# emiliofidalgo/liodom

Hardware: AMD Instinct MI355X
Metric: scans/sec (64×1800 cloud, prev_frames=20) at 1 GPU; pose RMSE vs CPU ref (higher is better)
Workload: dtype f64

## Files before the change

### liodom_amd/csrc/kernels_knn.h

```cpp
constexpr float kCellInv = 1.0f;
constexpr double kCellSize = 1.0;

struct Top5 {
  unsigned long long k0, k1, k2, k3, k4;
  int p0, p1, p2, p3, p4;
};
constexpr unsigned long long kTop5Empty = (0x7f800000ull << 32) | 0x7fffffffull;
__device__ __forceinline__ float top5_dist(unsigned long long k) { return __int_as_float((int)(k >> 32)); }
__device__ __forceinline__ int top5_index(unsigned long long k) { return (int)(unsigned int)(k & 0xFFFFFFFFull); }
#define TOP5_STAGE(K, P)                                          \
  {                                                               \
    const bool lt = ck < (K);                                     \
    const unsigned long long nk = lt ? ck : (K);                  \
    const int np = lt ? cp : (P);                                 \
    ck = lt ? (K) : ck;                                           \
    cp = lt ? (P) : cp;                                           \
    (K) = nk; (P) = np;                                           \
  }
__device__ __forceinline__ void top5_insert(Top5& t, float d, int wi, int pos) {
  unsigned long long ck = ((unsigned long long)(unsigned int)__float_as_int(d) << 32) | (unsigned int)wi;
  int cp = pos;
  if (ck < t.k4) {
    TOP5_STAGE(t.k0, t.p0)
    TOP5_STAGE(t.k1, t.p1)
// ... 125 lines not shown
      }
    }
    int adj[U];
#pragma unroll
    for (int u = 0; u < U; u++) adj[u] = s_adj[c[u]];
#pragma unroll
    for (int u = 0; u < U; u++) a[u] += adj[u];
    float4 m[U];
#pragma unroll
    for (int u = 0; u < U; u++) m[u] = sp[a[u]];
#pragma unroll
    for (int u = 0; u < U; u++)
      t.consider(i + u * kKnnGroup < T, sqdist_cand(qx, qy, qz, m[u]), __float_as_int(m[u].w), a[u]);
  }
  __builtin_amdgcn_wave_barrier();
  if (dbg && hl == 0) {
    dbg[0] = (unsigned int)(dbg_t1 - dbg_t0);
    dbg[1] = (unsigned int)(wall_clock64() - dbg_t1);
    dbg[2] = ((unsigned int)((T + U * kKnnGroup - 1) / (U * kKnnGroup)) << 16) | ((unsigned int)T << 20);
    dbg[3] = dbg_nseg;
  }
}

__device__ __forceinline__ bool best2_select(const Best2Acc& t, int hl, int half_shift, float& d5, int (&pos)[5]) {
  unsigned int v = (unsigned int)__float_as_int(t.m1), w = (unsigned int)__float_as_int(t.m2);
  int ph = t.p1, pn = t.p2;
  unsigned int g[6];
#pragma unroll
  for (int r = 0; r < 5; r++) {
    g[r] = half_min_u32(v);
    const unsigned int win = (unsigned int)((__ballot(v == g[r]) >> half_shift) & 0xFFFFFFFFull);
    const int l = __ffs(win) - 1;
    pos[r] = __shfl(ph, l, kKnnGroup);
    const bool mine = hl == l;
    v = mine ? w : v;
    w = mine ? 0x7f800000u : w;
    ph = mine ? pn : ph;
  }
  g[5] = half_min_u32(v);
  const unsigned int s3 = half_min_u32((unsigned int)__float_as_int(t.m3));
  const unsigned int one = 0x3f800000u;
  d5 = __int_as_float((int)g[4]);
  if (g[4] < one) return g[0] < g[1] && g[1] < g[2] && g[2] < g[3] && g[3] < g[4] && g[4] < g[5] && g[4] < s3;
  return s3 >= one;
}


__device__ __forceinline__ void knn_merge(Top5& t, Top5& g, int hl, int half_shift) {
  unsigned long long gk[5]; int gp[5];
#pragma unroll
  for (int r = 0; r < 5; r++) {
    const unsigned long long key = t.k0;
    const unsigned int dmin = half_min_u32((unsigned int)(key >> 32));
    unsigned int win = (unsigned int)((__ballot((unsigned int)(key >> 32) == dmin) >> half_shift) & 0xFFFFFFFFull);
    unsigned long long mk;
    if (__popc(win) == 1) {
      mk = ((unsigned long long)dmin << 32) | (unsigned int)__shfl((int)(unsigned int)(key & 0xFFFFFFFFull), __ffs(win) - 1, kKnnGroup);
    } else {
      mk = half_min_u64(key);
      win = (unsigned int)((__ballot(key == mk) >> half_shift) & 0xFFFFFFFFull);
    }
    const int wl = __ffs(win) - 1;
    gp[r] = __shfl(t.p0, wl, kKnnGroup);
    gk[r] = mk;
    if (hl == wl) {
      t.k0 = t.k1; t.k1 = t.k2; t.k2 = t.k3; t.k3 = t.k4; t.k4 = kTop5Empty;
      t.p0 = t.p1; t.p1 = t.p2; t.p2 = t.p3; t.p3 = t.p4; t.p4 = -1;
    }
  }
  g.k0 = gk[0]; g.k1 = gk[1]; g.k2 = gk[2]; g.k3 = gk[3]; g.k4 = gk[4];
  g.p0 = gp[0]; g.p1 = gp[1]; g.p2 = gp[2]; g.p3 = gp[3]; g.p4 = gp[4];
}

__device__ void rebuild_alloc(const DevView& v, int s, StreamState& st, int block, int nblocks);
__device__ void rebuild_count_and_pad(const DevView& v, int s, StreamState& st, int eb, int block, int* sbase, int* sslot, bool keep);

template <int kQ>
struct KnnShared {
  int incl[kQ][kKnnGroup];
  int adj[kQ][kKnnGroup];
  float nn[kQ][16];
  int res[kQ][4];
  double part[kQ][32];
  double blk[kQ][24];
};

__device__ __forceinline__ float best2_bound(const Best2Acc& t, int half_shift) {
  float B = 1.0f;
  const float thr[4] = {0.36f, 0.09f, 0.0225f, 0.0036f};
#pragma unroll
  for (int k = 0; k < 4; k++) {
    const int c = __popc((unsigned int)(__ballot(t.m1 <= thr[k]) >> half_shift)) + __popc((unsigned int)(__ballot(t.m2 <= thr[k]) >> half_shift));
    B = c >= 5 ? thr[k] : B;
  }
  return B;
}

template <class Tune>
__device__ __forceinline__ void knn_probe_cells(const DevView& v, const StreamState& st, int fc, int hl, int cx, int cy, int cz, float qx, float qy, float qz,
                                                const CellSlot* cells, const unsigned int* bits, unsigned int tmask,
                                                unsigned int& start, unsigned int& cnt, float& lb) {
  if (hl < 27) {
    const int dx = hl % 3 - 1, dy = (hl / 3) % 3 - 1, dz = hl / 9 - 1;
    const unsigned long long key = pack_cell(cx + dx, cy + dy, cz + dz);
    unsigned int h = hash_cell(key, tmask);
    if (Tune::kProbeBoth) {
      const unsigned int word = bits[h >> 5];
      const uint4 raw = *reinterpret_cast<const uint4*>(cells + h);
// ... 68 lines not shown
  const float r = fminf(sqrtf(pre.sq.w), 1.0f) + margin;
  const float B = r * r * (1.0f + 1e-5f);
  Top5Acc ta;
  {
    const unsigned long long sentinel = ((unsigned long long)(unsigned int)__float_as_int(B) << 32) | 0x7fffffffull;
    ta.t.k0 = ta.t.k1 = ta.t.k2 = ta.t.k3 = ta.t.k4 = sentinel;
    ta.t.p0 = ta.t.p1 = ta.t.p2 = ta.t.p3 = ta.t.p4 = -1;
  }
  const bool all = cnt > 0 && !(lb > B);
  knn_stream_cells<Top5Acc, 2, 2, 64>(ta, sp, sh.incl[grp], sh.adj[grp], start, all ? cnt : 0u, hl, qx, qy, qz);
  float gl = B;
  if (ta.t.p4 >= 0) gl = fminf(gl, top5_dist(ta.t.k4));
  pre.gsq = __int_as_float((int)half_min_u32((unsigned int)__float_as_int(gl)));
  pre.p[0] = ta.t.p0; pre.p[1] = ta.t.p1; pre.p[2] = ta.t.p2; pre.p[3] = ta.t.p3; pre.p[4] = ta.t.p4;
#pragma unroll
  for (int k = 0; k < 5; k++) pre.c[k] = sp[pre.p[k] >= 0 ? pre.p[k] : 0];
}

template <int kKnnThreads, bool kPre = false, bool kTail = true, bool kWt = kPre>
__device__ __forceinline__ void knn_block(const DevView& v, int s, StreamState& st, int fc, int outer_it, int eb, int bv, int E,
                                          KnnShared<kKnnThreads / kKnnGroup>& sh, const float4& p_in, const double (&T_in)[12],
                                          const KnnPre& pre, const double* qt) {
  constexpr int kKnnQueries = kKnnThreads / kKnnGroup;
  typedef KnnTune<(kKnnThreads >= 256)> Tune;
  const int grp = threadIdx.x / kKnnGroup;
  const int e = bv * kKnnQueries + grp;
  const int hl = threadIdx.x & (kKnnGroup - 1);
  const int half_shift = (threadIdx.x & 32);
  const bool dbgb = (bv == 5) && (s == 0) && (threadIdx.x == 0) && (outer_it == 0);
  const unsigned long long t_blk = (kInstrument && (v.debug & 32)) ? wall_clock64() : 0ull;
  DBG_STAMP(v, dbgb, 1, 0);
  bool active = e < E;
  float qx = 0.f, qy = 0.f, qz = 0.f;
  if (active) {
    float4 p = p_in;
    double T[12];
#pragma unroll
    for (int i = 0; i < 12; i++) T[i] = T_in[i];
    if (!Tune::kHoistLoads) {
      p = v.edges[((size_t)eb * v.n_streams + s) * v.edge_cap + e];
#pragma unroll
      for (int i = 0; i < 12; i++) T[i] = st.odom[i];
    }
    transform_point(T, p.x, p.y, p.z, &qx, &qy, &qz);
    if (v.knn_q && hl == 0) v.knn_q[((size_t)s * 2 + outer_it) * v.edge_cap + e] = make_float4(qx, qy, qz, 0.f);
    active = ld_isfinite((double)qx) && ld_isfinite((double)qy) && ld_isfinite((double)qz) &&
             fabsf(qx) < 1.0e9f && fabsf(qy) < 1.0e9f && fabsf(qz) < 1.0e9f;
  }
  DBG_STAMP(v, dbgb, 1, 1); DBG_QSTAMP(1);
  if (hl == 0) { sh.res[grp][0] = 0; sh.res[grp][1] = -1; sh.res[grp][2] = -1; }
  float d5 = __int_as_float(0x7f800000);
  if (active) {
    const int cx = (int)floorf(qx * kCellInv), cy = (int)floorf(qy * kCellInv), cz = (int)floorf(qz * kCellInv);
    const unsigned int tmask = st.table_mask;
    const int stab = s + LD_TAB_PARITY(v, fc) * v.n_streams;
    const CellSlot* cells = v.cells + (size_t)stab * v.table_size;
    const unsigned int* bits = v.cell_bits + (size_t)stab * (v.table_size >> 5);
    const float4* sp = v.sorted_pts + (size_t)stab * v.sorted_cap;
    float d5_r = __int_as_float(0x7f800000);
    int pos5[5] = {-1, -1, -1, -1, -1};
    bool reranked = false;
    if (kPre) {
      if ((kInstrument && (v.debug & 64)) && hl == 0 && !(pre.gsq > 0.f)) atomicAdd(&v.dbg_clk[262], 1ull);
      if (pre.gsq > 0.f) {
        Top5 t, g;
        top5_clear(t);
#pragma unroll
        for (int k = 0; k < 5; k++) {
          if (pre.p[k] >= 0) top5_insert(t, sqdist_f(qx, qy, qz, pre.c[k].x, pre.c[k].y, pre.c[k].z), __float_as_int(pre.c[k].w), pre.p[k]);
        }
        knn_merge(t, g, hl, half_shift);
        const float d5n = g.p4 >= 0 ? top5_dist(g.k4) : __int_as_float(0x7f800000);
        const double ddx = (double)qx - (double)pre.sq.x, ddy = (double)qy - (double)pre.sq.y, ddz = (double)qz - (double)pre.sq.z;
        const double delta = sqrt(ddx * ddx + ddy * ddy + ddz * ddz) * (1.0 + 1e-12);
        const double r = sqrt((double)pre.gsq) * (1.0 - 2e-7) - delta;
        double limit = r > 0.0 ? r * r * (1.0 - 1e-6) : 0.0;
        {
          const double cs = kCellSize;
          const double fx = (double)qx - (double)(int)floorf(pre.sq.x * kCellInv) * cs, fy = (double)qy - (double)(int)floorf(pre.sq.y * kCellInv) * cs,
                       fz = (double)qz - (double)(int)floorf(pre.sq.z * kCellInv) * cs;
          const double edge = fmin(fmin(fmin(fx, cs - fx), fmin(fy, cs - fy)), fmin(fz, cs - fz));
          const double ro = (cs + edge) * (1.0 - 2e-7);
          const double lo = ro > 0.0 ? ro * ro * (1.0 - 1e-6) : 0.0;
// ... 77 lines not shown
    Best2Acc b2;
    b2.clear();
    int dbg_n = 0;
    bool dbg_two_phase = false;
    {
      const bool now = pend && (have_b ? !(lb > B) : (hl == 13 || hl == 27 || lb <= Tune::kNearSq));
      if (kInstrument && (v.debug & 32)) dbg_n = __shfl(half_incl_scan_i32(now ? (int)cnt : 0), kKnnGroup - 1, kKnnGroup);
      knn_stream_cells<Best2Acc, Tune::kLoadsBig, Tune::kLoadsFlat, Tune::kBigCell, Tune::kCursor>(b2, sp, sh.incl[grp], sh.adj[grp], start, now ? cnt : 0u, hl, qx, qy, qz,
                                                                                     ((kInstrument && (v.debug & 32)) && s == 0 && e < E) ? v.dbg_q + ((size_t)outer_it * v.edge_cap + e) * 12 + 8 : nullptr);
      pend = pend && !now;
    }
    DBG_STAMP(v, dbgb, 1, 3); DBG_QSTAMP(3);
    if (!have_b && ((__ballot(pend) >> half_shift) & 0xFFFFFFFFull)) {
      B = best2_bound(b2, half_shift);
      pend = pend && !(lb > B);
      if ((__ballot(pend) >> half_shift) & 0xFFFFFFFFull) {
        if (kInstrument && (v.debug & 32)) { dbg_n += __shfl(half_incl_scan_i32(pend ? (int)cnt : 0), kKnnGroup - 1, kKnnGroup); dbg_two_phase = true; }
        knn_stream_cells<Best2Acc, Tune::kLoadsBig, Tune::kLoadsFlat, Tune::kBigCell, Tune::kCursor>(b2, sp, sh.incl[grp], sh.adj[grp], start, pend ? cnt : 0u, hl, qx, qy, qz);
      }
    } else {
      pend = false;
    }
    DBG_STAMP(v, dbgb, 1, 4); DBG_QSTAMP(4);
    const bool certain = best2_select(b2, hl, half_shift, d5, pos5) && !v.knn_exact_only;
    if ((kInstrument && (v.debug & 32)) && s == 0 && e < E && hl == 0) v.dbg_q[((size_t)outer_it * v.edge_cap + e) * 12] = (unsigned int)dbg_n | (dbg_two_phase ? 0x40000000u : 0u) | (certain ? 0u : 0x80000000u);
    if ((kInstrument && (v.debug & 64)) && hl == 0) {
      atomicAdd(&v.dbg_clk[256 + (certain ? 0 : 1)], 1ull);
      if (dbg_two_phase) atomicAdd(&v.dbg_clk[258], 1ull);
      atomicAdd(&v.dbg_clk[384 + (dbg_n / 64 < 63 ? dbg_n / 64 : 63)], 1ull);
    }
    if (!certain) {
      const bool all = cnt > 0 && (!(lb > B) || (!have_b && (hl == 13 || hl == 27 || lb <= Tune::kNearSq)));
      Top5Acc ta;
      Top5 g;
      {
        const float bnd = d5 < 1.0f ? d5 : 1.0f;
        const unsigned long long sentinel = ((unsigned long long)(unsigned int)__float_as_int(bnd) << 32) | 0x7fffffffull;
        ta.t.k0 = ta.t.k1 = ta.t.k2 = ta.t.k3 = ta.t.k4 = sentinel;
        ta.t.p0 = ta.t.p1 = ta.t.p2 = ta.t.p3 = ta.t.p4 = -1;
      }
      knn_stream_cells<Top5Acc, 2, 2, 64>(ta, sp, sh.incl[grp], sh.adj[grp], start, all ? cnt : 0u, hl, qx, qy, qz);
      knn_merge(ta.t, g, hl, half_shift);
      d5 = g.p4 >= 0 ? top5_dist(g.k4) : __int_as_float(0x7f800000);
      pos5[0] = g.p0; pos5[1] = g.p1; pos5[2] = g.p2; pos5[3] = g.p3; pos5[4] = g.p4;
    }
    if (outer_it == 0 && v.knn_save_pos && !(kWt && !kPre)) {
      const float sk = (cnt > 0 && !(!(lb > B) || (!have_b && (hl == 13 || hl == 27 || lb <= Tune::kNearSq)))) ? lb : __int_as_float(0x7f800000);
// ... 3 lines not shown
      float guard = __int_as_float((int)gd);
      {
        const float cs = (float)kCellSize;
        const float fx = qx - (float)cx * cs, fy = qy - (float)cy * cs, fz = qz - (float)cz * cs;
        float edge = fminf(fminf(fminf(fx, cs - fx), fminf(fy, cs - fy)), fminf(fz, cs - fz));
        edge = edge > 0.f ? edge : 0.f;
        const float outer = (cs + edge) * (cs + edge) * (1.0f - 1e-6f);
        guard = guard < outer ? guard : outer;
      }
      v.knn_save_pos[((size_t)s * v.edge_cap + e) * kKnnGroup + hl] = make_int2(b2.p1, b2.p2);
      if (hl == 0) v.knn_save_g[(size_t)s * v.edge_cap + e] = guard < 3.0e38f ? guard : 3.0e38f;
    }
    if ((kInstrument && (v.debug & 64)) && s == 0 && hl == 0) {
      const int bin = (int)((wall_clock64() - t_blk) / 100ull);
      atomicAdd(&v.dbg_clk[320 + (bin < 63 ? bin : 63)], 1ull);
      const int nb = dbg_n < 64 ? 0 : dbg_n < 128 ? 1 : dbg_n < 256 ? 2 : dbg_n < 512 ? 3 : dbg_n < 1024 ? 4 : 5;
      atomicAdd(&v.dbg_clk[448 + (bin / 4 < 7 ? bin / 4 : 7) * 8 + nb + (dbg_two_phase ? 0 : 0)], 1ull);
      if (!certain) atomicAdd(&v.dbg_clk[448 + (bin / 4 < 7 ? bin / 4 : 7) * 8 + 7], 1ull);
      if (dbg_two_phase) atomicAdd(&v.dbg_clk[448 + (bin / 4 < 7 ? bin / 4 : 7) * 8 + 6], 1ull);
    }
    }
    else d5 = d5_r;
    DBG_STAMP(v, dbgb, 1, 5); DBG_QSTAMP(5);
    if (d5 < 1.0f && !(kPre && reranked)) {
      const int mypos = hl == 0 ? pos5[0] : hl == 1 ? pos5[1] : hl == 2 ? pos5[2] : hl == 3 ? pos5[3] : pos5[4];
      if (hl < 5) {
        const float4 m = sp[mypos];
        sh.nn[grp][hl * 3 + 0] = m.x; sh.nn[grp][hl * 3 + 1] = m.y; sh.nn[grp][hl * 3 + 2] = m.z;
        if (hl < 2) sh.res[grp][1 + hl] = __float_as_int(m.w);
      }
      if (hl == 0) sh.res[grp][0] = 1;
    }
  }
  if (outer_it == 0 && v.knn_save_q && e < E && hl == 0) {
    v.knn_save_q[(size_t)s * v.edge_cap + e] = make_float4(qx, qy, qz, d5);
    if (!active && v.knn_save_g) v.knn_save_g[(size_t)s * v.edge_cap + e] = 0.f;
  }
  if (!kTail) return;
  __syncthreads();
  DBG_STAMP(v, dbgb, 1, 6); DBG_QSTAMP(6);
  if (kKnnThreads < 256 && v.knn_nn) {
    if (threadIdx.x < kKnnQueries * 5) {
      const int q = threadIdx.x / 5, j = threadIdx.x % 5;
      const int eq = bv * kKnnQueries + q;
      if (eq < v.edge_cap) {
        const int w = j == 0 ? sh.res[q][0] : (j == 1 ? sh.res[q][1] : (j == 2 ? sh.res[q][2] : 0));
        v.knn_nn[((size_t)s * v.edge_cap + eq) * 5 + j] = make_float4(sh.nn[q][j * 3], sh.nn[q][j * 3 + 1], sh.nn[q][j * 3 + 2], __int_as_float(w));
      }
    }
    return;
  }
  if (threadIdx.x < kKnnQueries) {
    const int q = threadIdx.x;
    const int eq = bv * kKnnQueries + q;
    bool valid = (eq < E) && (sh.res[q][0] != 0);
// ... 3 lines not shown
    if (valid) valid = line_gate(nx, ny, nz);
    if (eq < E) {
      float4* ca = v.corr_a + ((size_t)s * 2 + outer_it) * v.edge_cap + eq;
      float4* cb = v.corr_b + ((size_t)s * 2 + outer_it) * v.edge_cap + eq;
      int2* cidx = v.corr_idx + ((size_t)s * 2 + outer_it) * v.edge_cap + eq;
      const float4 oa = valid ? make_float4(nx[0], ny[0], nz[0], 1.0f) : make_float4(0, 0, 0, 0);
      const float4 ob = valid ? make_float4(nx[1], ny[1], nz[1], 0.0f) : make_float4(0, 0, 0, 0);
      const int2 oi = valid ? make_int2(sh.res[q][1], sh.res[q][2]) : make_int2(-1, -1);
      if (kWt) {
        wt_store_f4(ca, oa); wt_store_f4(cb, ob);
        wt_store_u64(cidx, ((unsigned long long)(unsigned int)oi.y << 32) | (unsigned int)oi.x);
      } else {
        *ca = oa; *cb = ob; *cidx = oi;
      }
    }
    const unsigned long long vb = __ballot(valid);
    const int nvalid = __popcll(vb);
    if (q == 0) {
      if (nvalid && !v.knn_partials) atomicAdd(&st.info.matches[outer_it], nvalid);
      unsigned char* cm = &v.corr_mask[((size_t)s * 2 + outer_it) * v.mask_stride + bv];
      if (kWt) wt_store_u8(cm, (unsigned char)vb); else *cm = (unsigned char)vb;
    }
    sh.res[q][3] = valid ? 1 : 0;
  } else if (kKnnThreads > 64 && v.knn_partials && threadIdx.x >= 64 && threadIdx.x < 64 + kKnnQueries) {
    const int q = threadIdx.x - 64;
    const int eq = bv * kKnnQueries + q;
    double flag = 0.0;
    if (eq < E && sh.res[q][0] != 0) {
      double Rm[12], pq[4], pt[3];
#pragma unroll
      for (int i = 0; i < 4; i++) pq[i] = kWt ? qt[i] : st.param_q[i];
#pragma unroll
      for (int i = 0; i < 3; i++) pt[i] = kWt ? qt[4 + i] : st.param_t[i];
      iso_from_qt(pq, pt, Rm);
      const float4 pe = v.edges[((size_t)eb * v.n_streams + s) * v.edge_cap + eq];
      const double p[3] = {(double)pe.x, (double)pe.y, (double)pe.z};
      const double a[3] = {(double)sh.nn[q][0], (double)sh.nn[q][1], (double)sh.nn[q][2]};
      const double b[3] = {(double)sh.nn[q][3], (double)sh.nn[q][4], (double)sh.nn[q][5]};
      double J[18], rs[3], rho0, rho1;
      const bool ok = residual_block(Rm, p, a, b, v.min_range, v.max_range, J, rs, &rho0, &rho1);
#pragma unroll
      for (int i = 0; i < 18; i++) sh.blk[q][i] = J[i];
      sh.blk[q][18] = rs[0]; sh.blk[q][19] = rs[1]; sh.blk[q][20] = rs[2]; sh.blk[q][21] = rho0; sh.blk[q][22] = rho1;
      flag = ok ? 1.0 : 2.0;
    }
    sh.blk[q][23] = flag;
  }
  if (!v.knn_partials) return;
  __syncthreads();
  if (hl < kAccN) {
    const double flag = sh.res[grp][3] ? sh.blk[grp][23] : 0.0;
    double x = 0.0;
    if (flag == 1.0) x = residual_entry(sh.blk[grp], sh.blk[grp] + 18, sh.blk[grp][21], sh.blk[grp][22], hl);
    else if (flag == 2.0 && hl == 28) x = 1.0;
    sh.part[grp][hl] = x;
  } else if (hl == kAccN) {
    sh.part[grp][hl] = sh.res[grp][3] ? 1.0 : 0.0;
  }
  __syncthreads();
  if (threadIdx.x <= kAccN) {
    double x = 0.0;
#pragma unroll
    for (int q = 0; q < kKnnQueries; q++) x += sh.part[q][threadIdx.x];
    double* dst = &v.knn_part[(((size_t)s * 2 + outer_it) * v.knn_blocks + bv) * 32 + threadIdx.x];
    if (kWt) wt_store_u64(dst, (unsigned long long)__double_as_longlong(x)); else *dst = x;
  }
  DBG_STAMP(v, dbgb, 1, 7); DBG_QSTAMP(7);
  if ((kInstrument && (v.debug & 64)) && s == 0 && threadIdx.x == 0) {
    const unsigned long long d = wall_clock64() - t_blk;
    const int bin = (int)(d / 100ull);
    atomicAdd(&v.dbg_clk[192 + (bin < 63 ? bin : 63)], 1ull);
  }
}

template <int kKnnThreads>
__device__ __forceinline__ void knn_tail_dual(const DevView& v, int s, int outer_it, int eb, int bvA, int bvB, bool haveB, int E,
                                              KnnShared<kKnnThreads / kKnnGroup>& shA, KnnShared<kKnnThreads / kKnnGroup>& shB, const double* qt) {
  constexpr int kKnnQueries = kKnnThreads / kKnnGroup;
  static_assert(kKnnThreads == 256, "two blocks of 8 queries on four waves");
  const int grp = threadIdx.x / kKnnGroup, hl = threadIdx.x & (kKnnGroup - 1);
  const int half = (int)threadIdx.x >> 7, t = (int)threadIdx.x & 127;
  KnnShared<kKnnQueries>& sh = half ? shB : shA;
  const int bv = half ? bvB : bvA;
  const bool live = half ? haveB : true;
  if (t < kKnnQueries && live) {
    const int q = t;
    const int eq = bv * kKnnQueries + q;
    bool valid = (eq < E) && (sh.res[q][0] != 0);
    float nx[5], ny[5], nz[5];
#pragma unroll
    for (int j = 0; j < 5; j++) { nx[j] = sh.nn[q][j * 3]; ny[j] = sh.nn[q][j * 3 + 1]; nz[j] = sh.nn[q][j * 3 + 2]; }
    if (valid) valid = line_gate(nx, ny, nz);
    if (eq < E) {
      const float4 oa = valid ? make_float4(nx[0], ny[0], nz[0], 1.0f) : make_float4(0, 0, 0, 0);
      const float4 ob = valid ? make_float4(nx[1], ny[1], nz[1], 0.0f) : make_float4(0, 0, 0, 0);
      const int2 oi = valid ? make_int2(sh.res[q][1], sh.res[q][2]) : make_int2(-1, -1);
      wt_store_f4(v.corr_a + ((size_t)s * 2 + outer_it) * v.edge_cap + eq, oa);
      wt_store_f4(v.corr_b + ((size_t)s * 2 + outer_it) * v.edge_cap + eq, ob);
      wt_store_u64(v.corr_idx + ((size_t)s * 2 + outer_it) * v.edge_cap + eq, ((unsigned long long)(unsigned int)oi.y << 32) | (unsigned int)oi.x);
    }
    const unsigned long long vb = __ballot(valid);
    if (q == 0) wt_store_u8(&v.corr_mask[((size_t)s * 2 + outer_it) * v.mask_stride + bv], (unsigned char)vb);
    sh.res[q][3] = valid ? 1 : 0;
  } else if (t >= 64 && t < 64 + kKnnQueries && live) {
    const int q = t - 64;
    const int eq = bv * kKnnQueries + q;
    double flag = 0.0;
    if (eq < E && sh.res[q][0] != 0) {
      double Rm[12], pq[4], pt[3];
#pragma unroll
      for (int i = 0; i < 4; i++) pq[i] = qt[i];
#pragma unroll
      for (int i = 0; i < 3; i++) pt[i] = qt[4 + i];
      iso_from_qt(pq, pt, Rm);
      const float4 pe = v.edges[((size_t)eb * v.n_streams + s) * v.edge_cap + eq];
      const double p[3] = {(double)pe.x, (double)pe.y, (double)pe.z};
      const double a[3] = {(double)sh.nn[q][0], (double)sh.nn[q][1], (double)sh.nn[q][2]};
      const double b[3] = {(double)sh.nn[q][3], (double)sh.nn[q][4], (double)sh.nn[q][5]};
      double J[18], rs[3], rho0, rho1;
      const bool ok = residual_block(Rm, p, a, b, v.min_range, v.max_range, J, rs, &rho0, &rho1);
#pragma unroll
      for (int i = 0; i < 18; i++) sh.blk[q][i] = J[i];
      sh.blk[q][18] = rs[0]; sh.blk[q][19] = rs[1]; sh.blk[q][20] = rs[2]; sh.blk[q][21] = rho0; sh.blk[q][22] = rho1;
      flag = ok ? 1.0 : 2.0;
    }
    sh.blk[q][23] = flag;
  }
  __syncthreads();
#pragma unroll
  for (int b = 0; b < 2; b++) {
    if (b == 1 && !haveB) break;
    KnnShared<kKnnQueries>& shb = b ? shB : shA;
    if (hl < kAccN) {
      const double flag = shb.res[grp][3] ? shb.blk[grp][23] : 0.0;
      double x = 0.0;
      if (flag == 1.0) x = residual_entry(shb.blk[grp], shb.blk[grp] + 18, shb.blk[grp][21], shb.blk[grp][22], hl);
      else if (flag == 2.0 && hl == 28) x = 1.0;
      shb.part[grp][hl] = x;
    } else if (hl == kAccN) {
      shb.part[grp][hl] = shb.res[grp][3] ? 1.0 : 0.0;
    }
  }
  __syncthreads();
  if (t <= kAccN && live) {
    double x = 0.0;
#pragma unroll
    for (int q = 0; q < kKnnQueries; q++) x += sh.part[q][t];
    wt_store_u64(&v.knn_part[(((size_t)s * 2 + outer_it) * v.knn_blocks + bv) * 32 + t], (unsigned long long)__double_as_longlong(x));
  }
}

__device__ __forceinline__ void chain_release_edges(const DevView& v, unsigned int signal_odo) {
  typedef __attribute__((address_space(1))) unsigned int gu32;
  if (signal_odo && threadIdx.x == 0) INJECT_DELAY(14);
  if (signal_odo && threadIdx.x == 0) __hip_atomic_store((gu32*)(v.pipe_flags + kEdgePipeBufs), signal_odo, __ATOMIC_RELAXED, __HIP_MEMORY_SCOPE_AGENT);
}

template <int kKnnThreads, bool kOv, bool kChain>
__device__ __forceinline__ bool knn_pass(const DevView& v, int s, int bxi, int byi, int outer_it, int eb, unsigned int wait_edges,
                                         unsigned int signal_odo, unsigned int seq, int scan_no, KnnShared<kKnnThreads / kKnnGroup>& sh, KnnShared<kKnnThreads / kKnnGroup>& sh2, double* sh_ov, int pred_copy = 0) {
  constexpr int kKnnQueries = kKnnThreads / kKnnGroup;
  static_assert(!(kOv && kChain), "the overlapped pass is the second pass, the chain-mode instance the first");
  StreamState& st = v.state[s];
  if (kOv) {
    if (!pipe_wait(v.ov_flags + s, seq, &st.status)) return false;
    OV_STAMP(v, threadIdx.x == 0 && bxi == 0, 9); OV_STAMP(v, threadIdx.x == 0 && bxi == v.knn_grid - 1, 13);
  } else if (kChain) {
    const bool pred_ok = pred_wait(v, s, bxi % kOvReplicas, (unsigned int)scan_no, sh_ov, &st.status, v.pipe_flags + eb, wait_edges, pred_copy);
    OV_STAMP(v, threadIdx.x == 0 && bxi == 0, 27);
    if (bxi == 0 && threadIdx.x == 0) { st.reb_frame_count = scan_no; st.n_used_tab[(scan_no + 1) & 1] = 0; st.reb_initialized = 1; st.cursor = 0; }
    if (pred_ok && bxi == 0 && threadIdx.x >= 64 && threadIdx.x < 76) st.pred_odom[scan_no & 1][threadIdx.x - 64] = sh_ov[threadIdx.x - 64];
    if (!pred_ok) return false;
// ... 7 lines not shown
  }
  if (!kOv && outer_it == 0) {
    if (!kChain && signal_odo && bxi == 0 && byi == 0 && threadIdx.x == 0) {
      typedef __attribute__((address_space(1))) unsigned int gu32;
      __hip_atomic_store((gu32*)(v.pipe_flags + kEdgePipeBufs), signal_odo, __ATOMIC_RELAXED, __HIP_MEMORY_SCOPE_AGENT);
    }
    if (!kChain && wait_edges && !pipe_wait(v.pipe_flags + eb, wait_edges, &st.status)) return false;
  }
  typedef KnnTune<(kKnnThreads >= 256)> Tune;
  const int e_first = bxi * kKnnQueries + (int)(threadIdx.x / kKnnGroup);
  float4 p_first = make_float4(0.f, 0.f, 0.f, 0.f);
  double T[12] = {0, 0, 0, 0, 0, 0, 0, 0, 0, 0, 0, 0};
  if (Tune::kHoistLoads) {
    p_first = v.edges[((size_t)eb * v.n_streams + s) * v.edge_cap + (e_first < v.edge_cap ? e_first : v.edge_cap - 1)];
    if (!kOv && !kChain) {
#pragma unroll
      for (int i = 0; i < 12; i++) T[i] = st.odom[i];
    }
  }
  if (kChain) {
#pragma unroll
    for (int i = 0; i < 12; i++) T[i] = sh_ov[i];
  }
  const unsigned int st_status = st.status;
  const int st_init = kChain ? 1 : st.initialized;
  const int fc = kChain ? scan_no : st.frame_count;
  int E;
  if (kChain) {
    typedef __attribute__((address_space(1))) unsigned int gu32;
    E = (int)__hip_atomic_load((gu32*)(v.edge_cnt + eb * 32 + s), __ATOMIC_RELAXED, __HIP_MEMORY_SCOPE_AGENT);
  } else {
    E = st.n_edges_buf[eb];
  }
  if (st_status & LIODOM_STATUS_PIPE_TIMEOUT) return false;
  if (!st_init) return true;
  static_assert(kKnnGridDiv == 2, "k_knn handles exactly two query blocks per workgroup");
  constexpr bool kWt = kOv || kChain;
  if (bxi * kKnnQueries >= E) {
    if (threadIdx.x == 0) {
      unsigned char* cm = &v.corr_mask[((size_t)s * 2 + outer_it) * v.mask_stride + bxi];
      if (kWt) wt_store_u8(cm, 0); else *cm = 0;
      if (bxi + v.knn_grid < v.knn_blocks) { if (kWt) wt_store_u8(cm + v.knn_grid, 0); else cm[v.knn_grid] = 0; }
    }
    return true;
  }
  const int bv2 = bxi + v.knn_grid;
  const int e_second = bv2 * kKnnQueries + (int)(threadIdx.x / kKnnGroup);
  const bool second = bv2 < v.knn_blocks && bv2 * kKnnQueries < E;
  KnnPre pre1, pre2;
  float4 p_second = make_float4(0.f, 0.f, 0.f, 0.f);
  if (kOv) {
    if (second) p_second = v.edges[((size_t)eb * v.n_streams + s) * v.edge_cap + (e_second < v.edge_cap ? e_second : v.edge_cap - 1)];
    knn_presearch<kKnnThreads>(v, s, st, fc, e_first, E, sh, pre1, sqrtf(p_first.x * p_first.x + p_first.y * p_first.y + p_first.z * p_first.z));
    if (second) knn_presearch<kKnnThreads>(v, s, st, fc, e_second, E, sh2, pre2, sqrtf(p_second.x * p_second.x + p_second.y * p_second.y + p_second.z * p_second.z));
    else pre2.gsq = 0.f;
    if (!ov_wait_pose(v, s, bxi % kOvReplicas, seq, sh_ov, &st.status)) return false;
    OV_STAMP(v, threadIdx.x == 0 && bxi == 0, 10); OV_STAMP(v, threadIdx.x == 0 && bxi == v.knn_grid - 1, 14);
    if (kInstrument && (v.debug & 128) && threadIdx.x == 0) {
      sh_ov[19] = __longlong_as_double((long long)wall_clock64());
      const unsigned long long pub = *(volatile unsigned long long*)&v.dbg_clk[448 + 1];
      const long long d = (long long)wall_clock64() - (long long)pub;
      if (pub && d >= 0) atomicAdd(&v.dbg_clk[320 + (d / 25 < 63 ? d / 25 : 63)], 1ull);
    }
#pragma unroll
    for (int i = 0; i < 12; i++) T[i] = sh_ov[i];
  }
  if constexpr (kOv) {
    knn_block<kKnnThreads, true, false>(v, s, st, fc, outer_it, eb, bxi, E, sh, p_first, T, pre1, sh_ov + 12);
    if (second) knn_block<kKnnThreads, true, false>(v, s, st, fc, outer_it, eb, bv2, E, sh2, p_second, T, pre2, sh_ov + 12);
    else if (bv2 < v.knn_blocks && threadIdx.x == 0) wt_store_u8(&v.corr_mask[((size_t)s * 2 + outer_it) * v.mask_stride + bv2], 0);
    __syncthreads();
    knn_tail_dual<kKnnThreads>(v, s, outer_it, eb, bxi, bv2, second, E, sh, sh2, sh_ov + 12);
    if (!v.speculate) return true;
    const int cf = ov_confirm_pose(v, s, bxi % kOvReplicas, seq, sh_ov, &st.status);
    if ((kInstrument && (v.debug & 64)) && threadIdx.x == 0) atomicAdd(&v.dbg_clk[271 + (cf == 1 ? 0 : 1)], 1ull);
    return cf == 1;
  }
  knn_block<kKnnThreads, false, true, kWt>(v, s, st, fc, outer_it, eb, bxi, E, sh, p_first, T, pre1, kChain ? sh_ov + 12 : nullptr);
  if (bv2 >= v.knn_blocks) return true;
  if (!second) {
    if (threadIdx.x == 0) { unsigned char* cm = &v.corr_mask[((size_t)s * 2 + outer_it) * v.mask_stride + bv2]; if (kWt) wt_store_u8(cm, 0); else *cm = 0; }
    return true;
  }
  __syncthreads();
  double T2[12] = {0, 0, 0, 0, 0, 0, 0, 0, 0, 0, 0, 0};
  if (Tune::kHoistLoads) {
    p_second = v.edges[((size_t)eb * v.n_streams + s) * v.edge_cap + (e_second < v.edge_cap ? e_second : v.edge_cap - 1)];
    asm volatile("" ::: "memory");
    if (kChain) {
#pragma unroll
      for (int i = 0; i < 12; i++) T2[i] = sh_ov[i];
// ... 85 lines not shown
  for (int i = 0; i < 19; i++) same = same && __double_as_longlong(sh_first[i]) == __double_as_longlong(sh_ov[i]);
  if (same) return;
  if (st.status & (LIODOM_STATUS_PIPE_TIMEOUT | LIODOM_STATUS_LM_SYNC_TIMEOUT)) return;
  if ((kInstrument && (v.debug & 64)) && threadIdx.x == 0) atomicAdd(&v.dbg_clk[273], 1ull);
  OV_STAMP(v, threadIdx.x == 0, 21);
  DevView vr = v;
  vr.knn_save_pos = nullptr;
  const int fc = st.frame_count;
  const int E = st.n_edges_buf[eb];
  const int outer_it = 1;
  if (!st.initialized || (st.status & LIODOM_STATUS_PIPE_TIMEOUT)) return;
  const int bv2 = bxi + v.knn_grid;
  if (bxi * kKnnQueries < E) {
    const bool second = bv2 < v.knn_blocks && bv2 * kKnnQueries < E;
    const float4* ed = v.edges + ((size_t)eb * v.n_streams + s) * v.edge_cap;
    const int e_first = bxi * kKnnQueries + (int)(threadIdx.x / kKnnGroup), e_second = bv2 * kKnnQueries + (int)(threadIdx.x / kKnnGroup);
    const float4 p_first = ed[e_first < v.edge_cap ? e_first : v.edge_cap - 1];
    const float4 p_second = ed[e_second < v.edge_cap ? e_second : v.edge_cap - 1];
    double T[12];
#pragma unroll
    for (int i = 0; i < 12; i++) T[i] = sh_ov[i];
    KnnPre none;
    none.gsq = 0.f;
    knn_block<kKnnThreads, false, false, true>(vr, s, st, fc, outer_it, eb, bxi, E, shs[0], p_first, T, none, sh_ov + 12);
    if (second) knn_block<kKnnThreads, false, false, true>(vr, s, st, fc, outer_it, eb, bv2, E, shs[1], p_second, T, none, sh_ov + 12);
    else if (bv2 < v.knn_blocks && threadIdx.x == 0) wt_store_u8(&v.corr_mask[((size_t)s * 2 + outer_it) * v.mask_stride + bv2], 0);
    __syncthreads();
    knn_tail_dual<kKnnThreads>(v, s, outer_it, eb, bxi, bv2, second, E, shs[0], shs[1], sh_ov + 12);
  }
  else return;
  if (scan_no >= 0) chain_count_done(v.knn_done0 + 32 + s); else ov_signal_knn_done(v, s, bxi, seq);
}

__global__ void k_ov_gate(DevView v, int s, unsigned int seq) {
  OV_STAMP(v, threadIdx.x == 0, 6);
  (void)pipe_wait(v.ov_flags + s, seq, &v.state[s].status);
  OV_STAMP(v, threadIdx.x == 0, 7);
}

template <bool kList = false>
__global__ __launch_bounds__(256) void k_line_gate(DevView v, int s0, int outer_it, int eb) {
  const int s = stream_of<kList>(v, s0, (int)blockIdx.y);
  StreamState& st = v.state[s];
  if (v.knn8_cnt && blockIdx.x == 0 && threadIdx.x == 0) v.knn8_cnt[s] = 0;
  if (!st.initialized) return;
  const int E = st.n_edges_buf[eb];
// ... 39 lines not shown
```

### liodom_amd/csrc/liodom_math.h

```cpp
#pragma once
#include <cfloat>
#include <cmath>
#include <cstdint>

#if defined(__HIPCC__)
#define LD_HD __host__ __device__ __forceinline__
#define LD_UNROLL _Pragma("unroll")
#define LD_FP_CONTRACT_FAST _Pragma("clang fp contract(fast)")
#else
#define LD_HD inline
#define LD_UNROLL
#define LD_FP_CONTRACT_FAST
#endif
#if defined(__HIP_DEVICE_COMPILE__)
#define LD_RSQRT(x) rsqrt(x)
#else
#define LD_RSQRT(x) (1.0 / sqrt(x))
#endif

namespace liodom_dev {

constexpr int kJacobiSweeps = 8;
constexpr int kLmMaxIterations = 4;
constexpr double kHuberA = 0.2;
// ... 440 lines not shown
    if (rho1 < DBL_MIN) rho1 = DBL_MIN;
  } else {
    rho0 = s; rho1 = 1.0;
  }
  double z = s * 0.0;
  LD_UNROLL
  for (int i = 0; i < 18; i++) z += J[i] * 0.0;
  *rho0_out = rho0; *rho1_out = rho1;
  rs[0] = rho1 * r0; rs[1] = rho1 * r1; rs[2] = rho1 * r2;
  return z == 0.0;
}
LD_HD double residual_entry(const double* J, const double* rs, double rho0, double rho1, int e) {
  LD_FP_CONTRACT_FAST
  if (e == 0) return 0.5 * rho0;
  if (e <= 6) { const int i = e - 1; return J[i] * rs[0] + J[6 + i] * rs[1] + J[12 + i] * rs[2]; }
  if (e >= 28) return 0.0;
  int k = e - 7, i = 0;
  while (k >= 6 - i) { k -= 6 - i; i++; }
  const int j = i + k;
  const double a0 = rho1 * J[i], a1 = rho1 * J[6 + i], a2 = rho1 * J[12 + i];
  return a0 * J[j] + a1 * J[6 + j] + a2 * J[12 + j];
}

LD_HD void residual_accumulate(const double* Rm , const double* p, const double* a,
                               const double* b, double min_d, double max_d, double* acc) {
  LD_FP_CONTRACT_FAST
  double J[18], rs[3], rho0, rho1;
  const bool ok = residual_block(Rm, p, a, b, min_d, max_d, J, rs, &rho0, &rho1);
  acc[28] += ok ? 0.0 : 1.0;
  acc[0] += ok ? 0.5 * rho0 : 0.0;
  if (!ok) return;
  LD_UNROLL
  for (int i = 0; i < 6; i++) {
    acc[1 + i] += J[i] * rs[0] + J[6 + i] * rs[1] + J[12 + i] * rs[2];
    const double a0 = rho1 * J[i], a1 = rho1 * J[6 + i], a2 = rho1 * J[12 + i];
    LD_UNROLL
    for (int j = i; j < 6; j++) acc[7 + h_idx(i, j)] += a0 * J[j] + a1 * J[6 + j] + a2 * J[12 + j];
  }
}

enum { LM_DONE = 0, LM_NEED_EVAL = 1 };
enum {
  LM_TERM_MAX_ITER = 0, LM_TERM_PARAM_TOL = 1, LM_TERM_FUNC_TOL = 2, LM_TERM_GRAD_TOL = 3,
  LM_TERM_NO_RESIDUALS = 4, LM_TERM_EVAL_FAILURE = 5, LM_TERM_RADIUS = 6, LM_TERM_INVALID_STEPS = 7
};

// ... 405 lines not shown
```

Measured before the change: 14840.

## Hand over KNN neighbours directly and column-reduce residual partials in shared memory

For large KNN blocks, the lanes that already hold the winning neighbour candidates write them straight into shared memory during best-2 selection. This skips the separate gather of the five positions from sorted points. The start pose matrix and each query's edge point are now cached in shared memory, so the residual threads no longer rebuild the rotation from the quaternion or reload the edge from global memory. The per-query partial buffer plus its extra barrier is replaced by per-column sums computed from the stored Jacobian blocks by threads mapped to one wave per column group. This adds recomputation per column and some new debug stamps.

```diff
diff --git a/liodom_amd/csrc/kernels_knn.h b/liodom_amd/csrc/kernels_knn.h
--- a/liodom_amd/csrc/kernels_knn.h
+++ b/liodom_amd/csrc/kernels_knn.h
@@ -171,10 +171,13 @@
   }
 }
 
-__device__ __forceinline__ bool best2_select(const Best2Acc& t, int hl, int half_shift, float& d5, int (&pos)[5]) {
+template <bool kRank>
+__device__ __forceinline__ bool best2_select_t(const Best2Acc& t, int hl, int half_shift, float& d5, int (&pos)[5], int& r1, int& r2) {
   unsigned int v = (unsigned int)__float_as_int(t.m1), w = (unsigned int)__float_as_int(t.m2);
   int ph = t.p1, pn = t.p2;
   unsigned int g[6];
+  int pops = 0;
+  if (kRank) { r1 = -1; r2 = -1; }
 #pragma unroll
   for (int r = 0; r < 5; r++) {
     g[r] = half_min_u32(v);
@@ -182,6 +185,11 @@
     const int l = __ffs(win) - 1;
     pos[r] = __shfl(ph, l, kKnnGroup);
     const bool mine = hl == l;
+    if (kRank) {
+      r2 = (mine && pops == 1) ? r : r2;
+      r1 = (mine && pops == 0) ? r : r1;
+      pops += mine ? 1 : 0;
+    }
     v = mine ? w : v;
     w = mine ? 0x7f800000u : w;
     ph = mine ? pn : ph;
@@ -192,6 +200,10 @@
   d5 = __int_as_float((int)g[4]);
   if (g[4] < one) return g[0] < g[1] && g[1] < g[2] && g[2] < g[3] && g[3] < g[4] && g[4] < g[5] && g[4] < s3;
   return s3 >= one;
+}
+__device__ __forceinline__ bool best2_select(const Best2Acc& t, int hl, int half_shift, float& d5, int (&pos)[5]) {
+  int r1, r2;
+  return best2_select_t<false>(t, hl, half_shift, d5, pos, r1, r2);
 }
 
 
@@ -224,7 +236,9 @@
 __device__ void rebuild_alloc(const DevView& v, int s, StreamState& st, int block, int nblocks);
 __device__ void rebuild_count_and_pad(const DevView& v, int s, StreamState& st, int eb, int block, int* sbase, int* sslot, bool keep);
 
-template <int kQ>
+#define KNN_STAMP_LANDED(v, cond, i) do { if (kInstrument && ((v).debug & 32) && (cond)) { __builtin_amdgcn_s_waitcnt(0); (v).dbg_clk[32 + (i)] = wall_clock64(); } } while (0)
+
+template <int kQ, bool kFew = (kQ * kKnnGroup >= 256)>
 struct KnnShared {
   int incl[kQ][kKnnGroup];
   int adj[kQ][kKnnGroup];
@@ -233,6 +247,62 @@
   double part[kQ][32];
   double blk[kQ][24];
 };
+template <int kQ>
+struct KnnShared<kQ, true> {
+  int incl[kQ][kKnnGroup];
+  int adj[kQ][kKnnGroup];
+  float nn[kQ][16];
+  int res[kQ][4];
+  float4 edge[kQ];
+  double Rm[12];
+  double blk[kQ][24];
+};
+template <int kQ>
+__device__ __forceinline__ double knn_column_sum(const KnnShared<kQ, true>& sh, int c) {
+  double flag[kQ];
+#pragma unroll
+  for (int q = 0; q < kQ; q++) flag[q] = sh.res[q][3] ? sh.blk[q][23] : 0.0;
+  double x = 0.0;
+  if (c == 0) {
+#pragma unroll
+    for (int q = 0; q < kQ; q++) { const double v = residual_entry(sh.blk[q], sh.blk[q] + 18, sh.blk[q][21], sh.blk[q][22], 0); x += flag[q] == 1.0 ? v : 0.0; }
+  } else if (c <= 6) {
+#pragma unroll
+    for (int q = 0; q < kQ; q++) { const double v = residual_entry_g(sh.blk[q], sh.blk[q] + 18, c - 1); x += flag[q] == 1.0 ? v : 0.0; }
+  } else if (c < 28) {
+    int i, j;
+    residual_entry_ij(c, &i, &j);
+#pragma unroll
+    for (int q = 0; q < kQ; q++) { const double v = residual_entry_h(sh.blk[q], sh.blk[q][22], i, j); x += flag[q] == 1.0 ? v : 0.0; }
+  } else if (c == 28) {
+#pragma unroll
+    for (int q = 0; q < kQ; q++) x += flag[q] == 2.0 ? 1.0 : 0.0;
+  } else {
+#pragma unroll
+    for (int q = 0; q < kQ; q++) x += sh.res[q][3] ? 1.0 : 0.0;
+  }
+  return x;
+}
+template <int kWaves>
+__device__ __forceinline__ int knn_column_of(int t) {
+  const int w = t >> 6, l = t & 63;
+  if (l > kAccN) return -1;
+  const int cw = (l >= 7 && l < 28) ? 0 : (kWaves >= 3 ? (l >= 1 && l <= 6 ? 1 : 2) : 1);
+  return w == cw ? l : -1;
+}
+template <int kQ>
+__device__ __forceinline__ void knn_put_start_pose(KnnShared<kQ, true>& sh, const double* q, const double* t) {
+  double pq[4], pt[3], Rm[12];
+#pragma unroll
+  for (int i = 0; i < 4; i++) pq[i] = q[i];
+#pragma unroll
+  for (int i = 0; i < 3; i++) pt[i] = t[i];
+  iso_from_qt(pq, pt, Rm);
+#pragma unroll
+  for (int i = 0; i < 12; i++) sh.Rm[i] = Rm[i];
+}
+template <int kQ>
+__device__ __forceinline__ void knn_put_start_pose(KnnShared<kQ, false>&, const double*, const double*) {}
 
 __device__ __forceinline__ float best2_bound(const Best2Acc& t, int half_shift) {
   float B = 1.0f;
@@ -347,6 +417,8 @@
                                           KnnShared<kKnnThreads / kKnnGroup>& sh, const float4& p_in, const double (&T_in)[12],
                                           const KnnPre& pre, const double* qt) {
   constexpr int kKnnQueries = kKnnThreads / kKnnGroup;
+  constexpr bool kFew = kKnnThreads >= 256;
+  constexpr bool kHandOver = kFew && kTail && !kPre;
   typedef KnnTune<(kKnnThreads >= 256)> Tune;
   const int grp = threadIdx.x / kKnnGroup;
   const int e = bv * kKnnQueries + grp;
@@ -374,6 +446,7 @@
   }
   DBG_STAMP(v, dbgb, 1, 1); DBG_QSTAMP(1);
   if (hl == 0) { sh.res[grp][0] = 0; sh.res[grp][1] = -1; sh.res[grp][2] = -1; }
+  if constexpr (kFew) { if (hl == 0) sh.edge[grp] = p_in; }
   float d5 = __int_as_float(0x7f800000);
   if (active) {
     const int cx = (int)floorf(qx * kCellInv), cy = (int)floorf(qy * kCellInv), cz = (int)floorf(qz * kCellInv);
@@ -384,6 +457,7 @@
     const float4* sp = v.sorted_pts + (size_t)stab * v.sorted_cap;
     float d5_r = __int_as_float(0x7f800000);
     int pos5[5] = {-1, -1, -1, -1, -1};
+    bool handed = false;
     bool reranked = false;
     if (kPre) {
       if ((kInstrument && (v.debug & 64)) && hl == 0 && !(pre.gsq > 0.f)) atomicAdd(&v.dbg_clk[262], 1ull);
@@ -507,7 +581,24 @@
       pend = false;
     }
     DBG_STAMP(v, dbgb, 1, 4); DBG_QSTAMP(4);
-    const bool certain = best2_select(b2, hl, half_shift, d5, pos5) && !v.knn_exact_only;
+    float4 c1 = make_float4(0.f, 0.f, 0.f, 0.f), c2 = c1;
+    int r1 = -1, r2 = -1;
+    if constexpr (kHandOver) { c1 = sp[b2.p1 >= 0 ? b2.p1 : 0]; c2 = sp[b2.p2 >= 0 ? b2.p2 : 0]; }
+    const bool certain = (kHandOver ? best2_select_t<true>(b2, hl, half_shift, d5, pos5, r1, r2) : best2_select(b2, hl, half_shift, d5, pos5)) && !v.knn_exact_only;
+    if constexpr (kHandOver) {
+      if (certain && d5 < 1.0f) {
+        if (r1 >= 0) {
+          sh.nn[grp][r1 * 3 + 0] = c1.x; sh.nn[grp][r1 * 3 + 1] = c1.y; sh.nn[grp][r1 * 3 + 2] = c1.z;
+          if (r1 < 2) sh.res[grp][1 + r1] = __float_as_int(c1.w);
+        }
+        if (r2 >= 0) {
+          sh.nn[grp][r2 * 3 + 0] = c2.x; sh.nn[grp][r2 * 3 + 1] = c2.y; sh.nn[grp][r2 * 3 + 2] = c2.z;
+          if (r2 < 2) sh.res[grp][1 + r2] = __float_as_int(c2.w);
+        }
+        if (hl == 0) sh.res[grp][0] = 1;
+        handed = true;
+      }
+    }
     if ((kInstrument && (v.debug & 32)) && s == 0 && e < E && hl == 0) v.dbg_q[((size_t)outer_it * v.edge_cap + e) * 12] = (unsigned int)dbg_n | (dbg_two_phase ? 0x40000000u : 0u) | (certain ? 0u : 0x80000000u);
     if ((kInstrument && (v.debug & 64)) && hl == 0) {
       atomicAdd(&v.dbg_clk[256 + (certain ? 0 : 1)], 1ull);
@@ -557,7 +648,7 @@
     }
     else d5 = d5_r;
     DBG_STAMP(v, dbgb, 1, 5); DBG_QSTAMP(5);
-    if (d5 < 1.0f && !(kPre && reranked)) {
+    if (d5 < 1.0f && !(kPre && reranked) && !handed) {
       const int mypos = hl == 0 ? pos5[0] : hl == 1 ? pos5[1] : hl == 2 ? pos5[2] : hl == 3 ? pos5[3] : pos5[4];
       if (hl < 5) {
         const float4 m = sp[mypos];
@@ -566,6 +657,7 @@
       }
       if (hl == 0) sh.res[grp][0] = 1;
     }
+    KNN_STAMP_LANDED(v, dbgb, 8);
   }
   if (outer_it == 0 && v.knn_save_q && e < E && hl == 0) {
     v.knn_save_q[(size_t)s * v.edge_cap + e] = make_float4(qx, qy, qz, d5);
@@ -615,18 +707,27 @@
       if (kWt) wt_store_u8(cm, (unsigned char)vb); else *cm = (unsigned char)vb;
     }
     sh.res[q][3] = valid ? 1 : 0;
+    KNN_STAMP_LANDED(v, dbgb, 9);
   } else if (kKnnThreads > 64 && v.knn_partials && threadIdx.x >= 64 && threadIdx.x < 64 + kKnnQueries) {
     const int q = threadIdx.x - 64;
     const int eq = bv * kKnnQueries + q;
     double flag = 0.0;
     if (eq < E && sh.res[q][0] != 0) {
-      double Rm[12], pq[4], pt[3];
-#pragma unroll
-      for (int i = 0; i < 4; i++) pq[i] = kWt ? qt[i] : st.param_q[i];
-#pragma unroll
-      for (int i = 0; i < 3; i++) pt[i] = kWt ? qt[4 + i] : st.param_t[i];
-      iso_from_qt(pq, pt, Rm);
-      const float4 pe = v.edges[((size_t)eb * v.n_streams + s) * v.edge_cap + eq];
+      double Rm[12];
+      float4 pe;
+      if constexpr (kFew) {
+#pragma unroll
+        for (int i = 0; i < 12; i++) Rm[i] = sh.Rm[i];
+        pe = sh.edge[q];
+      } else {
+        double pq[4], pt[3];
+#pragma unroll
+        for (int i = 0; i < 4; i++) pq[i] = kWt ? qt[i] : st.param_q[i];
+#pragma unroll
+        for (int i = 0; i < 3; i++) pt[i] = kWt ? qt[4 + i] : st.param_t[i];
+        iso_from_qt(pq, pt, Rm);
+        pe = v.edges[((size_t)eb * v.n_streams + s) * v.edge_cap + eq];
+      }
       const double p[3] = {(double)pe.x, (double)pe.y, (double)pe.z};
       const double a[3] = {(double)sh.nn[q][0], (double)sh.nn[q][1], (double)sh.nn[q][2]};
       const double b[3] = {(double)sh.nn[q][3], (double)sh.nn[q][4], (double)sh.nn[q][5]};
@@ -638,9 +739,19 @@
       flag = ok ? 1.0 : 2.0;
     }
     sh.blk[q][23] = flag;
+    KNN_STAMP_LANDED(v, (bv == 5) && (s == 0) && (threadIdx.x == 64) && (outer_it == 0), 10);
   }
   if (!v.knn_partials) return;
   __syncthreads();
+  if constexpr (kFew) {
+    DBG_STAMP(v, dbgb, 1, 12);
+    const int col = knn_column_of<kKnnThreads / kWave>((int)threadIdx.x);
+    if (col >= 0) {
+      const double x = knn_column_sum(sh, col);
+      double* dst = &v.knn_part[(((size_t)s * 2 + outer_it) * v.knn_blocks + bv) * 32 + col];
+      if (kWt) wt_store_u64(dst, (unsigned long long)__double_as_longlong(x)); else *dst = x;
+    }
+  } else {
   if (hl < kAccN) {
     const double flag = sh.res[grp][3] ? sh.blk[grp][23] : 0.0;
     double x = 0.0;
@@ -657,6 +768,7 @@
     for (int q = 0; q < kKnnQueries; q++) x += sh.part[q][threadIdx.x];
     double* dst = &v.knn_part[(((size_t)s * 2 + outer_it) * v.knn_blocks + bv) * 32 + threadIdx.x];
     if (kWt) wt_store_u64(dst, (unsigned long long)__double_as_longlong(x)); else *dst = x;
+  }
   }
   DBG_STAMP(v, dbgb, 1, 7); DBG_QSTAMP(7);
   if ((kInstrument && (v.debug & 64)) && s == 0 && threadIdx.x == 0) {
@@ -676,6 +788,8 @@
   KnnShared<kKnnQueries>& sh = half ? shB : shA;
   const int bv = half ? bvB : bvA;
   const bool live = half ? haveB : true;
+  const bool dbgt = (bvA == 5) && (s == 0);
+  DBG_STAMP(v, dbgt && threadIdx.x == 0, 1, 18);
   if (t < kKnnQueries && live) {
     const int q = t;
     const int eq = bv * kKnnQueries + q;
@@ -695,18 +809,16 @@
     const unsigned long long vb = __ballot(valid);
     if (q == 0) wt_store_u8(&v.corr_mask[((size_t)s * 2 + outer_it) * v.mask_stride + bv], (unsigned char)vb);
     sh.res[q][3] = valid ? 1 : 0;
+    KNN_STAMP_LANDED(v, dbgt && threadIdx.x == 0, 19);
   } else if (t >= 64 && t < 64 + kKnnQueries && live) {
     const int q = t - 64;
     const int eq = bv * kKnnQueries + q;
     double flag = 0.0;
     if (eq < E && sh.res[q][0] != 0) {
-      double Rm[12], pq[4], pt[3];
-#pragma unroll
-      for (int i = 0; i < 4; i++) pq[i] = qt[i];
-#pragma unroll
-      for (int i = 0; i < 3; i++) pt[i] = qt[4 + i];
-      iso_from_qt(pq, pt, Rm);
-      const float4 pe = v.edges[((size_t)eb * v.n_streams + s) * v.edge_cap + eq];
+      double Rm[12];
+#pragma unroll
+      for (int i = 0; i < 12; i++) Rm[i] = shA.Rm[i];
+      const float4 pe = sh.edge[q];
       const double p[3] = {(double)pe.x, (double)pe.y, (double)pe.z};
       const double a[3] = {(double)sh.nn[q][0], (double)sh.nn[q][1], (double)sh.nn[q][2]};
       const double b[3] = {(double)sh.nn[q][3], (double)sh.nn[q][4], (double)sh.nn[q][5]};
@@ -718,29 +830,16 @@
       flag = ok ? 1.0 : 2.0;
     }
     sh.blk[q][23] = flag;
+    KNN_STAMP_LANDED(v, dbgt && threadIdx.x == 64, 20);
   }
   __syncthreads();
-#pragma unroll
-  for (int b = 0; b < 2; b++) {
-    if (b == 1 && !haveB) break;
-    KnnShared<kKnnQueries>& shb = b ? shB : shA;
-    if (hl < kAccN) {
-      const double flag = shb.res[grp][3] ? shb.blk[grp][23] : 0.0;
-      double x = 0.0;
-      if (flag == 1.0) x = residual_entry(shb.blk[grp], shb.blk[grp] + 18, shb.blk[grp][21], shb.blk[grp][22], hl);
-      else if (flag == 2.0 && hl == 28) x = 1.0;
-      shb.part[grp][hl] = x;
-    } else if (hl == kAccN) {
-      shb.part[grp][hl] = shb.res[grp][3] ? 1.0 : 0.0;
-    }
-  }
-  __syncthreads();
-  if (t <= kAccN && live) {
-    double x = 0.0;
-#pragma unroll
-    for (int q = 0; q < kKnnQueries; q++) x += sh.part[q][t];
-    wt_store_u64(&v.knn_part[(((size_t)s * 2 + outer_it) * v.knn_blocks + bv) * 32 + t], (unsigned long long)__double_as_longlong(x));
-  }
+  DBG_STAMP(v, dbgt && threadIdx.x == 0, 1, 21);
+  const int col = knn_column_of<2>(t);
+  if (col >= 0 && live) {
+    const double x = knn_column_sum(sh, col);
+    wt_store_u64(&v.knn_part[(((size_t)s * 2 + outer_it) * v.knn_blocks + bv) * 32 + col], (unsigned long long)__double_as_longlong(x));
+  }
+  KNN_STAMP_LANDED(v, dbgt && threadIdx.x == 0, 22);
 }
 
 __device__ __forceinline__ void chain_release_edges(const DevView& v, unsigned int signal_odo) {
@@ -794,6 +893,9 @@
 #pragma unroll
     for (int i = 0; i < 12; i++) T[i] = sh_ov[i];
   }
+  if constexpr (kKnnThreads >= 256 && !kOv) {
+    if (threadIdx.x == kKnnThreads - 1) knn_put_start_pose(sh, kChain ? sh_ov + 12 : st.param_q, kChain ? sh_ov + 16 : st.param_t);
+  }
   const unsigned int st_status = st.status;
   const int st_init = kChain ? 1 : st.initialized;
   const int fc = kChain ? scan_no : st.frame_count;
@@ -828,6 +930,7 @@
     else pre2.gsq = 0.f;
     if (!ov_wait_pose(v, s, bxi % kOvReplicas, seq, sh_ov, &st.status)) return false;
     OV_STAMP(v, threadIdx.x == 0 && bxi == 0, 10); OV_STAMP(v, threadIdx.x == 0 && bxi == v.knn_grid - 1, 14);
+    DBG_STAMP(v, bxi == 5 && s == 0 && threadIdx.x == 0, 1, 16);
     if (kInstrument && (v.debug & 128) && threadIdx.x == 0) {
       sh_ov[19] = __longlong_as_double((long long)wall_clock64());
       const unsigned long long pub = *(volatile unsigned long long*)&v.dbg_clk[448 + 1];
@@ -836,9 +939,11 @@
     }
 #pragma unroll
     for (int i = 0; i < 12; i++) T[i] = sh_ov[i];
+    if (threadIdx.x == 127) knn_put_start_pose(sh, sh_ov + 12, sh_ov + 16);
   }
   if constexpr (kOv) {
     knn_block<kKnnThreads, true, false>(v, s, st, fc, outer_it, eb, bxi, E, sh, p_first, T, pre1, sh_ov + 12);
+    KNN_STAMP_LANDED(v, bxi == 5 && s == 0 && threadIdx.x == 0, 17);
     if (second) knn_block<kKnnThreads, true, false>(v, s, st, fc, outer_it, eb, bv2, E, sh2, p_second, T, pre2, sh_ov + 12);
     else if (bv2 < v.knn_blocks && threadIdx.x == 0) wt_store_u8(&v.corr_mask[((size_t)s * 2 + outer_it) * v.mask_stride + bv2], 0);
     __syncthreads();
@@ -970,6 +1075,7 @@
     for (int i = 0; i < 12; i++) T[i] = sh_ov[i];
     KnnPre none;
     none.gsq = 0.f;
+    if (threadIdx.x == 127) knn_put_start_pose(shs[0], sh_ov + 12, sh_ov + 16);
     knn_block<kKnnThreads, false, false, true>(vr, s, st, fc, outer_it, eb, bxi, E, shs[0], p_first, T, none, sh_ov + 12);
     if (second) knn_block<kKnnThreads, false, false, true>(vr, s, st, fc, outer_it, eb, bv2, E, shs[1], p_second, T, none, sh_ov + 12);
     else if (bv2 < v.knn_blocks && threadIdx.x == 0) wt_store_u8(&v.corr_mask[((size_t)s * 2 + outer_it) * v.mask_stride + bv2], 0);
diff --git a/liodom_amd/csrc/liodom_math.h b/liodom_amd/csrc/liodom_math.h
--- a/liodom_amd/csrc/liodom_math.h
+++ b/liodom_amd/csrc/liodom_math.h
@@ -486,6 +486,21 @@
   return a0 * J[j] + a1 * J[6 + j] + a2 * J[12 + j];
 }
 
+LD_HD void residual_entry_ij(int e, int* i_out, int* j_out) {
+  int k = e - 7, i = 0;
+  while (k >= 6 - i) { k -= 6 - i; i++; }
+  *i_out = i; *j_out = i + k;
+}
+LD_HD double residual_entry_g(const double* J, const double* rs, int i) {
+  LD_FP_CONTRACT_FAST
+  return J[i] * rs[0] + J[6 + i] * rs[1] + J[12 + i] * rs[2];
+}
+LD_HD double residual_entry_h(const double* J, double rho1, int i, int j) {
+  LD_FP_CONTRACT_FAST
+  const double a0 = rho1 * J[i], a1 = rho1 * J[6 + i], a2 = rho1 * J[12 + i];
+  return a0 * J[j] + a1 * J[6 + j] + a2 * J[12 + j];
+}
+
 LD_HD void residual_accumulate(const double* Rm , const double* p, const double* a,
                                const double* b, double min_d, double max_d, double* acc) {
   LD_FP_CONTRACT_FAST
```

Result: no change. 14730 (-0.8%).
